# wei-zeng98/piano-a2s

Measured on AMD Instinct MI355X. Metric: training clips/sec (12 s, 5-bar), higher is better.
Workload: dtype f32

## Files before the change

### include/a2s.h

```cpp
#ifndef A2S_H
#define A2S_H
#include <stddef.h>
#include <stdint.h>
#ifdef __cplusplus
extern "C" {
#endif

#define A2S_OK 0
#define A2S_ERR_ARG (-1)
#define A2S_ERR_HIP (-2)
#define A2S_ERR_WORKSPACE (-3)

const char* a2s_last_error(void);
int a2s_version(void);
long long a2s_launch_count(void);

int a2s_gemm_f32(void* stream, int M, int N, int K, float alpha, const float* A, long sAm, long sAk,
                 const float* B, long sBk, long sBn, float beta, float* C, long ldc, const float* bias, int act,
                 int batch, long bsA, long bsB, long bsC, int splitk, float* workspace, size_t workspace_bytes);
int a2s_gemm_f32_affine(void* stream, int M, int N, int K, float alpha, const float* A, long sAm, long sAk, const float* B, long sBk,
                        long sBn, float beta, float* C, long ldc, const float* bias, int act, int batch, long bsA, long bsB, long bsC,
                        int splitk, float* workspace, size_t workspace_bytes, const float* a_scale, const float* a_shift, int a_period,
                        const float* b_scale, const float* b_shift, int b_period);
int a2s_gemm_f32_bnstats(void* stream, int M, int N, int K, const float* A, long sAm, long sAk, const float* B, long sBk, long sBn, float* C, long ldc,
                         const float* y, const float* mean, const float* invstd, const float* scale, const float* shift, int period, float* partial);
int a2s_gemm_f32_affine_scaled(void* stream, int M, int N, int K, float alpha, const float* A, long sAm, long sAk, const float* B, long sBk,
                               long sBn, float beta, float* C, long ldc, const float* bias, int act, int batch, long bsA, long bsB, long bsC,
                               int splitk, float* workspace, size_t workspace_bytes, const float* a_scale, const float* a_shift, int a_period,
                               const float* b_scale, const float* b_shift, int b_period, const float* a_absmax, const float* b_absmax);
int a2s_gemm_f32_bnstats_scaled(void* stream, int M, int N, int K, const float* A, long sAm, long sAk, const float* B, long sBk, long sBn, float* C, long ldc,
                                const float* y, const float* mean, const float* invstd, const float* scale, const float* shift, int period, float* partial,
                                const float* a_absmax, const float* b_absmax);
int a2s_linear_dgrad_bnstats(void* stream, int M, int N, int K, const float* dz, long lda, const float* Wt, float* da, long ldc, const float* y,
                             const float* mean, const float* invstd, const float* scale, const float* shift, int period, float* partial,
                             const float* dz_absmax, const float* w_absmax, float* workspace, size_t workspace_bytes, float* da_absmax_out);
int a2s_linear_fwd(void* stream, int M, int N, int K, const float* y, long lda, const float* W, float* z, long ldc, const float* scale, const float* shift,
                   int period, const float* y_absmax, const float* w_absmax, float* workspace, size_t workspace_bytes);
int a2s_linear_fwd_eligible(int M, int N, int K, int period);
int a2s_linear_wgrad(void* stream, int M, int N, int K, const float* dz, long ldz, const float* y, long lda, float* G, long ldg, const float* scale,
                     const float* shift, int period, const float* dz_absmax, const float* y_absmax, float* workspace, size_t workspace_bytes);
size_t a2s_linear_wgrad_ws_bytes(int M, int K);
int a2s_linear_wgrad_eligible(int M, int N, int K, int period);
int a2s_tallk_wgrad(void* stream, int M, int Np, int K, const float* P, long ldp, const float* A, long lda, float* G, long ldg, int transposed, float* bias,
                    const float* p_absmax, const float* a_absmax, float* workspace, size_t workspace_bytes);
size_t a2s_tallk_wgrad_ws_bytes(int M, int Np, int K);
int a2s_tallk_wgrad_eligible(int M, int Np, int K, long ldp, long lda, long ldg, int transposed);
size_t a2s_linear_dgrad_ws_bytes(int N, int K);
int a2s_linear_dgrad_blocks(int M);
int a2s_linear_dgrad_eligible(int M, int N, int K, int period);
int a2s_absmax(void* stream, const float* x, long n, float* out);
int a2s_gemm_bnstats_blocks(int M, int period);
size_t a2s_gemm_workspace_bytes(int M, int N, int batch, int splitk);
int a2s_gemm_pick_splitk(int M, int N, int K, int batch);
void a2s_gemm_debug_tile(int cfg);
int a2s_debug_set(const char* key, int value);
int a2s_debug_get(const char* key);
int a2s_env_check(void);
int a2s_persist_abort_latch(void* device_word);

int a2s_conv3x3(void* stream, const float* x, const float* w, float* y, const float* in_scale, const float* in_shift,
                float* stat_partial, int B, int T, int F, int Cin, int Cout, int flip, float* workspace);
int a2s_conv3x3_ranged(void* stream, const float* x, const float* w, float* y, const float* in_scale, const float* in_shift, const float* in_absmax,
                       float* stat_partial, float* out_absmax, int B, int T, int F, int Cin, int Cout, float* workspace);
int a2s_conv3x3_stat_blocks(int B, int T, int F, int Cin);
int a2s_conv3x3_dgrad_bnstats(void* stream, const float* dy, const float* w, float* g, const float* yl, const float* yl_mean, const float* yl_invstd,
                              const float* yl_scale, const float* yl_shift, float* stat_partial, int B, int T, int F, int Cin, int Cout,
                              float* workspace);
int a2s_bn_bwd_from_partial(void* stream, const float* g, const float* x, const float* mean, const float* invstd, const float* scale, const float* shift,
                            float* dgamma, float* dbeta, float* dx , const float* partial, int nblocks, float* c12, long rows, int C, int F);
int a2s_conv3x3_dgrad_bnstats_scaled(void* stream, const float* dy, const float* w, float* g, const float* yl, const float* yl_mean, const float* yl_invstd,
                                     const float* yl_scale, const float* yl_shift, float* stat_partial, int B, int T, int F, int Cin, int Cout,
                                     float* workspace, const float* dy_absmax);
int a2s_conv3x3_dgrad_bnstats_ranged(void* stream, const float* dy, const float* w, float* g, const float* yl, const float* yl_mean, const float* yl_invstd,
                                     const float* yl_scale, const float* yl_shift, float* stat_partial, int B, int T, int F, int Cin, int Cout,
                                     float* workspace, const float* dy_absmax, float* g_absmax_out);
int a2s_bn_bwd_from_partial_amax(void* stream, const float* g, const float* x, const float* mean, const float* invstd, const float* scale, const float* shift,
                                 float* dgamma, float* dbeta, float* dx, const float* partial, int nblocks, float* c12, long rows, int C, int F,
                                 float* dx_absmax);
size_t a2s_conv3x3_workspace_floats(int Cin);
// ... 300 lines not shown
```

### piano_a2s_amd/csrc/a2s_api.hip

```cpp
#define A2S_SWITCHES_IMPL
#include "a2s_internal.h"

thread_local char a2s_err_msg[512] = {0};
long long a2s_launch_counter = 0;

#define ST ((hipStream_t)stream)

extern "C" {

const char* a2s_last_error(void) { return a2s_err_msg; }
int a2s_version(void) { return 1; }
long long a2s_launch_count(void) { return __atomic_load_n(&a2s_launch_counter, __ATOMIC_RELAXED); }

int a2s_gemm_f32(void* stream, int M, int N, int K, float alpha, const float* A, long sAm, long sAk, const float* B, long sBk,
                 long sBn, float beta, float* C, long ldc, const float* bias, int act, int batch, long bsA, long bsB, long bsC,
                 int splitk, float* workspace, size_t workspace_bytes) {
    return a2s_gemm_impl(ST, M, N, K, alpha, A, sAm, sAk, B, sBk, sBn, beta, C, ldc, bias, act, batch, bsA, bsB, bsC, splitk,
                         workspace, workspace_bytes);
}
int a2s_gemm_f32_affine(void* stream, int M, int N, int K, float alpha, const float* A, long sAm, long sAk, const float* B, long sBk,
                        long sBn, float beta, float* C, long ldc, const float* bias, int act, int batch, long bsA, long bsB, long bsC,
                        int splitk, float* workspace, size_t workspace_bytes, const float* a_scale, const float* a_shift, int a_period,
                        const float* b_scale, const float* b_shift, int b_period) {
    return a2s_gemm_affine_impl(ST, M, N, K, alpha, A, sAm, sAk, B, sBk, sBn, beta, C, ldc, bias, act, batch, bsA, bsB, bsC, splitk,
// ... 7 lines not shown
    return a2s_gemm_affine_impl(ST, M, N, K, alpha, A, sAm, sAk, B, sBk, sBn, beta, C, ldc, bias, act, batch, bsA, bsB, bsC, splitk,
                                workspace, workspace_bytes, a_scale, a_shift, a_period, b_scale, b_shift, b_period,
                                nullptr, nullptr, nullptr, nullptr, nullptr, nullptr, 0, 1, a_absmax, b_absmax);
}
int a2s_gemm_f32_bnstats_scaled(void* stream, int M, int N, int K, const float* A, long sAm, long sAk, const float* B, long sBk, long sBn, float* C, long ldc,
                                const float* y, const float* mean, const float* invstd, const float* scale, const float* shift, int period, float* partial,
                                const float* a_absmax, const float* b_absmax) {
    return a2s_gemm_affine_impl(ST, M, N, K, 1.f, A, sAm, sAk, B, sBk, sBn, 0.f, C, ldc, nullptr, 0, 1, 0, 0, 0, 1, nullptr, 0,
                                nullptr, nullptr, 0, nullptr, nullptr, 0, y, mean, invstd, scale, shift, partial, period, 1, a_absmax, b_absmax);
}
int a2s_absmax(void* stream, const float* x, long n, float* out) { return a2s_absmax_impl(ST, x, n, out); }
int a2s_linear_dgrad_bnstats(void* stream, int M, int N, int K, const float* dz, long lda, const float* Wt, float* da, long ldc, const float* y,
                             const float* mean, const float* invstd, const float* scale, const float* shift, int period, float* partial,
                             const float* dz_absmax, const float* w_absmax, float* workspace, size_t workspace_bytes, float* da_absmax_out) {
    return a2s_linear_dgrad_bnstats_impl(ST, M, N, K, dz, lda, Wt, 1, K, da, ldc, y, mean, invstd, scale, shift, period, partial, dz_absmax, w_absmax,
                                         workspace, workspace_bytes, da_absmax_out);
}
size_t a2s_linear_dgrad_ws_bytes(int N, int K) { return a2s_linear_dgrad_ws_bytes_impl(N, K); }
int a2s_linear_fwd(void* stream, int M, int N, int K, const float* y, long lda, const float* W, float* z, long ldc, const float* scale, const float* shift,
                   int period, const float* y_absmax, const float* w_absmax, float* workspace, size_t workspace_bytes) {
    return a2s_linear_fwd_impl(ST, M, N, K, y, lda, W, z, ldc, scale, shift, period, y_absmax, w_absmax, workspace, workspace_bytes);
}
int a2s_linear_wgrad(void* stream, int M, int N, int K, const float* dz, long ldz, const float* y, long lda, float* G, long ldg, const float* scale,
                     const float* shift, int period, const float* dz_absmax, const float* y_absmax, float* workspace, size_t workspace_bytes) {
    return a2s_linear_wgrad_impl(ST, M, N, K, dz, ldz, y, lda, G, ldg, scale, shift, period, dz_absmax, y_absmax, workspace, workspace_bytes);
}
size_t a2s_linear_wgrad_ws_bytes(int M, int K) { return a2s_linear_wgrad_ws_bytes_impl(M, K); }
int a2s_linear_wgrad_eligible(int M, int N, int K, int period) { return a2s_linear_wgrad_ok(M, N, K, 256, 4, 4, period, nullptr, nullptr, nullptr) ? 1 : 0; }
int a2s_tallk_wgrad(void* stream, int M, int Np, int K, const float* P, long ldp, const float* A, long lda, float* G, long ldg, int transposed, float* bias,
                    const float* p_absmax, const float* a_absmax, float* workspace, size_t workspace_bytes) {
    return a2s_tallk_wgrad_impl(ST, M, Np, K, P, ldp, A, lda, G, ldg, transposed, bias, p_absmax, a_absmax, workspace, workspace_bytes);
}
size_t a2s_tallk_wgrad_ws_bytes(int M, int Np, int K) { return a2s_tallk_wgrad_ws_bytes_impl(M, Np, K); }
int a2s_tallk_wgrad_eligible(int M, int Np, int K, long ldp, long lda, long ldg, int transposed) {
    return a2s_tallk_wgrad_ok(M, Np, K, ldp, lda, ldg, transposed, nullptr, nullptr, nullptr, nullptr) ? 1 : 0;
}
int a2s_linear_fwd_eligible(int M, int N, int K, int period) { return a2s_linear_fwd_ok(M, N, K, 4, 4, period, nullptr, nullptr, nullptr) ? 1 : 0; }
int a2s_linear_dgrad_blocks(int M) { return a2s_linear_dgrad_blocks_impl(M); }
int a2s_linear_dgrad_eligible(int M, int N, int K, int period) {
    return a2s_linear_dgrad_ok(M, N, K, 4, 1, K, 4, period, nullptr, nullptr, nullptr, nullptr) ? 1 : 0;
}
int a2s_gemm_f32_bnstats(void* stream, int M, int N, int K, const float* A, long sAm, long sAk, const float* B, long sBk, long sBn, float* C, long ldc,
                         const float* y, const float* mean, const float* invstd, const float* scale, const float* shift, int period, float* partial) {
    return a2s_gemm_affine_impl(ST, M, N, K, 1.f, A, sAm, sAk, B, sBk, sBn, 0.f, C, ldc, nullptr, 0, 1, 0, 0, 0, 1, nullptr, 0,
                                nullptr, nullptr, 0, nullptr, nullptr, 0, y, mean, invstd, scale, shift, partial, period, 0, nullptr, nullptr);
}
int a2s_gemm_bnstats_blocks(int M, int period) { return a2s_cdiv(M, 128) * a2s_gemm_bnstats_slots(period); }
size_t a2s_gemm_workspace_bytes(int M, int N, int batch, int splitk) { return a2s_gemm_workspace_bytes_impl(M, N, batch, splitk); }
int a2s_gemm_pick_splitk(int M, int N, int K, int batch) { return a2s_gemm_pick_splitk_impl(M, N, K, batch); }
void a2s_gemm_debug_tile(int cfg) { a2s_gemm_debug_tile_impl(cfg); }
size_t a2s_note_step_workspace_floats(int H, int E) { return a2s_note_step_workspace_floats_impl(H, E); }
int a2s_debug_set(const char* key, int value) {
    if (!key) return A2S_ERR_ARG;
    const int id = a2s_switch_find(key);
    if (id >= 0) { a2s_switch_store(id, value); return A2S_OK; }
    if (!strcmp(key, "attn_deferred_fast")) { a2s_attn_deferred_fast = value ? 1 : 0; return A2S_OK; }
    if (!strcmp(key, "tallk_wgrad")) { a2s_tallk_wgrad_on = value ? 1 : 0; return A2S_OK; }
    if (!strcmp(key, "tallk_wgrad_max_splits")) { a2s_tallk_wgrad_max_splits = value > 0 ? value : 0; return A2S_OK; }
    if (!strcmp(key, "gemm_tile")) { a2s_gemm_debug_tile_impl(value); return A2S_OK; }
    snprintf(a2s_err_msg, sizeof(a2s_err_msg), "a2s_debug_set: unknown key %s", key);
    return A2S_ERR_ARG;
}
int a2s_env_check(void) {
    if (const char* e = a2s_switch_env_error()) A2S_FAIL(A2S_ERR_ARG, "%s: expected a decimal number >= 0", e);
    return A2S_OK;
}

int a2s_persist_abort_latch(void* device_word) { a2s_persist_latch_set(device_word); return A2S_OK; }

int a2s_debug_get(const char* key) {
    if (!key) return -1;
    const int id = a2s_switch_find(key);
    if (id == A2S_SW_attn_pair_fused_rows) return a2s_attn_pair_fused_rows();
    if (id >= 0) return a2s_sw((a2s_switch)id);
    if (!strcmp(key, "attn_pair_launches")) return (int)a2s_attn_pair_launches();
    if (!strcmp(key, "attn_pair_bwd_launches")) return (int)a2s_attn_pair_bwd_launches();
    if (!strcmp(key, "attn_deferred_fast")) return a2s_attn_deferred_fast;
    if (!strcmp(key, "tallk_wgrad")) return a2s_tallk_wgrad_on;
    if (!strcmp(key, "tallk_wgrad_max_splits")) return a2s_tallk_wgrad_max_splits;
    if (!strcmp(key, "tallk_wgrad_launches")) return (int)a2s_tallk_wgrad_launches();
    if (!strcmp(key, "attn_dk_ahead_launches")) return (int)a2s_attn_dk_ahead_launches();
    if (!strcmp(key, "attn_denc_launches")) return (int)a2s_attn_denc_launches();
    if (!strcmp(key, "dec_mid_launches")) return a2s_dec_mid_launches();
    if (!strcmp(key, "dec_cmb_launches")) return a2s_dec_cmb_launches();
    if (!strcmp(key, "dec_persist_launches")) return a2s_dec_persist_launches();
    if (!strcmp(key, "edit_distance_launches")) return (int)a2s_edit_distance_launches();
    if (!strcmp(key, "conv_rows16_c20_launches")) return (int)a2s_conv_rows16_c20_launches();
    if (!strcmp(key, "device_cus")) return a2s_device_geometry().cus;
    if (!strcmp(key, "device_xccs")) return a2s_device_geometry().xccs;
    return -1;
}

int a2s_conv3x3(void* stream, const float* x, const float* w, float* y, const float* in_scale, const float* in_shift,
                float* stat_partial, int B, int T, int F, int Cin, int Cout, int flip, float* workspace) {
    return a2s_conv3x3_impl(ST, x, w, y, in_scale, in_shift, stat_partial, B, T, F, Cin, Cout, flip, workspace, nullptr, nullptr, nullptr, nullptr, nullptr, nullptr,
                            nullptr, nullptr);
}
int a2s_conv3x3_ranged(void* stream, const float* x, const float* w, float* y, const float* in_scale, const float* in_shift, const float* in_absmax,
                       float* stat_partial, float* out_absmax, int B, int T, int F, int Cin, int Cout, float* workspace) {
    return a2s_conv3x3_impl(ST, x, w, y, in_scale, in_shift, stat_partial, B, T, F, Cin, Cout, 0, workspace, nullptr, nullptr, nullptr, nullptr, nullptr, nullptr,
                            in_absmax, out_absmax);
}
int a2s_conv3x3_dgrad_bnstats(void* stream, const float* dy, const float* w, float* g, const float* yl, const float* yl_mean, const float* yl_invstd,
                              const float* yl_scale, const float* yl_shift, float* stat_partial, int B, int T, int F, int Cin, int Cout,
                              float* workspace) {
    if (!yl) { snprintf(a2s_err_msg, sizeof(a2s_err_msg), "conv3x3_dgrad_bnstats: yl is required"); return A2S_ERR_ARG; }
    return a2s_conv3x3_impl(ST, dy, w, g, nullptr, nullptr, stat_partial, B, T, F, Cin, Cout, 1, workspace, yl, yl_mean, yl_invstd, yl_scale, yl_shift, nullptr, nullptr, nullptr);
}
int a2s_conv3x3_dgrad_bnstats_scaled(void* stream, const float* dy, const float* w, float* g, const float* yl, const float* yl_mean, const float* yl_invstd,
                                     const float* yl_scale, const float* yl_shift, float* stat_partial, int B, int T, int F, int Cin, int Cout,
                                     float* workspace, const float* dy_absmax) {
    if (!yl) { snprintf(a2s_err_msg, sizeof(a2s_err_msg), "conv3x3_dgrad_bnstats_scaled: yl is required"); return A2S_ERR_ARG; }
    return a2s_conv3x3_impl(ST, dy, w, g, nullptr, nullptr, stat_partial, B, T, F, Cin, Cout, 1, workspace, yl, yl_mean, yl_invstd, yl_scale, yl_shift, dy_absmax, nullptr, nullptr);
// ... 384 lines not shown
```

### piano_a2s_amd/csrc/a2s_internal.h

```cpp
#pragma once
#include "a2s_common.h"
#include "../../include/a2s.h"
#include "a2s_switches.h"

static inline int a2s_attn_pair_fused_rows(void) {
    const int cap = a2s_sw(A2S_SW_dec_fused_max_rows), v = a2s_sw(A2S_SW_attn_pair_fused_rows);
    return v < cap ? v : cap;
}
static inline unsigned a2s_persist_dbg(void) {
    return (a2s_sw(A2S_SW_persist_force_agent) ? PERSIST_DBG_FORCE_AGENT : 0u) | (a2s_sw(A2S_SW_persist_inject_abort) ? PERSIST_DBG_INJECT_ABORT : 0u);
}

int a2s_absmax_impl(hipStream_t st, const float* x, long n, float* out);
size_t a2s_gemm_workspace_bytes_impl(int M, int N, int batch, int splitk);
int a2s_gemm_pick_splitk_impl(int M, int N, int K, int batch);
int a2s_gemm_bnstats_slots(int period);
void a2s_gemm_debug_tile_impl(int cfg);
int a2s_gemm_affine_impl(hipStream_t st, int M, int N, int K, float alpha, const float* A, long sAm, long sAk,
    const float* B, long sBk, long sBn, float beta, float* C, long ldc, const float* bias, int act,
    int batch, long bsA, long bsB, long bsC, int splitk, float* ws, size_t ws_bytes,
    const float* a_scale, const float* a_shift, int a_period, const float* b_scale, const float* b_shift, int b_period,
    const float* ep_y, const float* ep_mean, const float* ep_invstd, const float* ep_scale, const float* ep_shift,
    float* ep_partial, int ep_period, int two_term, const float* a_absmax, const float* b_absmax);
int a2s_gemm_impl(hipStream_t st, int M, int N, int K, float alpha, const float* A, long sAm, long sAk,
    const float* B, long sBk, long sBn, float beta, float* C, long ldc, const float* bias, int act,
    int batch, long bsA, long bsB, long bsC, int splitk, float* ws, size_t ws_bytes);

size_t a2s_linear_dgrad_ws_bytes_impl(int N, int K);
int a2s_linear_dgrad_blocks_impl(int M);
bool a2s_linear_dgrad_ok(int M, int N, int K, long lda, long sBk, long sBn, long ldc, int period, const void* A, const void* B, const void* C, const void* y);
int a2s_linear_dgrad_bnstats_impl(hipStream_t st, int M, int N, int K, const float* A, long lda, const float* Wt, long sBk, long sBn, float* C, long ldc,
    const float* ep_y, const float* mean, const float* invstd, const float* scale, const float* shift, int period,
    float* partial, const float* a_absmax, const float* b_absmax, float* ws, size_t ws_bytes, float* c_absmax_out);
bool a2s_linear_fwd_ok(int M, int N, int K, long lda, long ldc, int period, const void* A, const void* W, const void* C);
int a2s_linear_fwd_impl(hipStream_t st, int M, int N, int K, const float* A, long lda, const float* W, float* C, long ldc, const float* a_scale,
    const float* a_shift, int period, const float* a_absmax, const float* w_absmax, float* ws, size_t ws_bytes);
size_t a2s_linear_wgrad_ws_bytes_impl(int M, int K);
bool a2s_linear_wgrad_ok(int M, int N, int K, long ldz, long lda, long ldg, int period, const void* dz, const void* A, const void* G);
int a2s_linear_wgrad_impl(hipStream_t st, int M, int N, int K, const float* dz, long ldz, const float* A, long lda, float* G, long ldg, const float* a_scale,
    const float* a_shift, int period, const float* dz_absmax, const float* a_absmax, float* ws, size_t ws_bytes);
extern int a2s_tallk_wgrad_on;
extern int a2s_tallk_wgrad_max_splits;
long a2s_tallk_wgrad_launches(void);
size_t a2s_tallk_wgrad_ws_bytes_impl(int M, int Np, int K);
bool a2s_tallk_wgrad_ok(int M, int Np, int K, long ldp, long lda, long ldg, int transposed, const void* P, const void* A, const void* G, const void* bias);
int a2s_tallk_wgrad_impl(hipStream_t st, int M, int Np, int K, const float* P, long ldp, const float* A, long lda, float* G, long ldg, int transposed,
    float* bias, const float* p_absmax, const float* a_absmax, float* ws, size_t ws_bytes);

int a2s_act_bound_impl(hipStream_t st, const float* scale, const float* shift, const float* absmax, int C, float* out);
size_t a2s_conv3x3_workspace_floats_impl(int Cin);
int a2s_conv3x3_impl(hipStream_t st, const float* x, const float* w, float* y, const float* in_scale,
    const float* in_shift, float* stat_partial, int B, int T, int F, int Cin, int Cout, int flip, float* ws,
    const float* yl, const float* yl_mean, const float* yl_invstd, const float* yl_scale, const float* yl_shift,
    const float* x_absmax, const float* in_absmax, float* out_absmax);
int a2s_conv3x3_stat_blocks_impl(int B, int T, int F, int Cin);
int a2s_bn_finalize_impl(hipStream_t st, const float* partial, int nblocks, int C, double count, const float* gamma,
    const float* beta, float* running_mean, float* running_var, long long* nbt, float* mean,
    float* invstd, float* scale, float* shift, float eps, float momentum, int training);
int a2s_bn_relu_apply_impl(hipStream_t st, const float* x, float* y, const float* scale, const float* shift, long n, int C, int F);
int a2s_col_stats_impl(hipStream_t st, const float* x, float* partial, long rows, int C, int rows_per_block);
int a2s_bn1d_relu_dropout_impl(hipStream_t st, const float* x, float* y, const float* scale, const float* shift,
    const uint8_t* mask, float inv_keep, long n, int C);
size_t a2s_conv3x3_wgrad_workspace_bytes_impl(int Cin, int Cout);
int a2s_conv3x3_wgrad_impl(hipStream_t st, const float* dy, const float* x, const float* in_scale, const float* in_shift, float* dW,
    float* ws, size_t ws_bytes, int B, int T, int F, int Cin, int Cout, const float* bn_y, const float* bn_mean,
    const float* bn_invstd, const float* bn_scale, const float* bn_shift, const float* bn_c12, float* dy_out,
    const float* dy_absmax, const float* act_absmax);
int a2s_bn_bwd_impl(hipStream_t st, const float* g, const float* x, const float* mean, const float* invstd, const float* scale,
    const float* shift, const uint8_t* mask, float inv_keep, float* dgamma, float* dbeta, float* dx, float* partial,
    float* c12, long rows, int C, int F, float* dx_absmax);
int a2s_bn_bwd_from_partial_impl(hipStream_t st, const float* g, const float* x, const float* mean, const float* invstd, const float* scale,
    const float* shift, float* dgamma, float* dbeta, float* dx, const float* partial, int nblocks, float* c12,
    long rows, int C, int F, float* dx_absmax);
int a2s_bn_bwd_stats_impl(hipStream_t st, const float* g, const float* x, const float* mean, const float* invstd, const float* scale,
    const float* shift, const uint8_t* mask, float inv_keep, float* partial, float* sums, long rows, int C, int F);
int a2s_bn_bwd_apply_impl(hipStream_t st, const float* g, const float* x, const float* mean, const float* invstd, const float* scale,
// ... 305 lines not shown
```

### piano_a2s_amd/csrc/a2s_linear.hip

```cpp
#include "a2s_internal.h"

#define LIN_BM 128
#define LIN_K 256
#define LIN_RS 288
#define LIN_NTH 512
#define LIN_LDS (2 * 2 * LIN_BM * LIN_RS)

typedef unsigned lu32x4 __attribute__((ext_vector_type(4)));

struct LinDgradArgs {
    const float* A; long lda;
    const unsigned char* planes;
    float* C; long ldc;
    const float* ep_y;
    const float* mean; const float* invstd; const float* scale; const float* shift;
    float* partial;
    const float* a_absmax; const float* b_absmax;
    int M, N, period, channels;
    float* c_absmax_out;
};

__global__ __launch_bounds__(256) void lin_pack_planes_k(const float* __restrict__ W, long ld, int N, int K, const float* __restrict__ absmax,
                                                         unsigned char* __restrict__ out) {
    const long id = (long)blockIdx.x * 256 + threadIdx.x;
// ... 580 lines not shown
    if (M < 1 || K < LIN_BM || K % LIN_BM) return 0;
    const size_t nsteps = 2 * (size_t)((M + 63) / 64);
    return nsteps * 16 * 2 * 1024 + (size_t)lin_wgrad_splits(M, K) * 256 * K * sizeof(float);
}
bool a2s_linear_wgrad_ok(int M, int N, int K, long ldz, long lda, long ldg, int period, const void* dz, const void* A, const void* G) {
    return N == 256 && M >= 64 && K >= LIN_BM && K % LIN_BM == 0 && (period == 0 || (period % 4 == 0 && K % period == 0)) && lda % 4 == 0 && ldg % 4 == 0 && ldz >= 256 &&
           (((uintptr_t)dz | (uintptr_t)A | (uintptr_t)G) % 16 == 0);
}
int a2s_linear_wgrad_impl(hipStream_t st, int M, int N, int K, const float* dz, long ldz, const float* A, long lda, float* G, long ldg, const float* a_scale,
                          const float* a_shift, int period, const float* dz_absmax, const float* a_absmax, float* ws, size_t ws_bytes) {
    A2S_REQUIRE(dz && A && G && dz_absmax && ws && ((a_scale == nullptr) == (a_shift == nullptr)), "linear_wgrad: null argument");
    A2S_REQUIRE(a2s_linear_wgrad_ok(M, N, K, ldz, lda, ldg, a_scale ? period : 0, dz, A, G), "linear_wgrad: needs N = 256, K %% 128 == 0, period %% 4 == 0, 16-byte aligned rows");
    A2S_REQUIRE(((uintptr_t)ws % 16 == 0) && ws_bytes >= a2s_linear_wgrad_ws_bytes_impl(M, K), "linear_wgrad: workspace too small (%zu bytes needed)",
                a2s_linear_wgrad_ws_bytes_impl(M, K));
    const int nblk = (M + 63) / 64, nsteps = 2 * nblk, splits = lin_wgrad_splits(M, K);
    unsigned char* planes = reinterpret_cast<unsigned char*>(ws);
    float* partial = reinterpret_cast<float*>(planes + (size_t)nsteps * 16 * 2 * 1024);
    hipLaunchKernelGGL(lin_pack_dz_planes, dim3((unsigned)(((long)nsteps * 1024 + 255) / 256)), dim3(256), 0, st, dz, ldz, M, nsteps, dz_absmax, planes);
    A2S_CHECK_LAUNCH("lin_pack_dz_planes");
    LinWgradArgs a{A, lda, planes, partial, a_scale, a_shift, a_absmax, dz_absmax, M, K, a_scale ? period : K, nblk, (nblk + splits - 1) / splits, 0, 256, nullptr};
    hipLaunchKernelGGL(lin_wgrad_roles<false>, dim3(K / LIN_BM, splits), dim3(LIN_NTH), 0, st, a);
    A2S_CHECK_LAUNCH("lin_wgrad");
    const long n = 256L * K;
    hipLaunchKernelGGL(lin_wgrad_reduce<false>, dim3((unsigned)((n / 4 + 255) / 256)), dim3(256), 0, st, partial, splits, n, G, ldg, K, nullptr, nullptr);
    A2S_CHECK_LAUNCH("lin_wgrad_reduce");
    return A2S_OK;
}

#define TALLK_SLAB_BYTES (64u << 20)
int a2s_tallk_wgrad_on = 1;
int a2s_tallk_wgrad_max_splits = 0;
static long long g_tallk_launches = 0;
long a2s_tallk_wgrad_launches(void) { return (long)__atomic_load_n(&g_tallk_launches, __ATOMIC_RELAXED); }

static int tallk_splits(int M, int Np, int K) {
    const int tiles = (K / LIN_BM) * (Np / 256), nblk = (M + 63) / 64;
    int cus = a2s_device_geometry().cus;
    if (cus < 1) cus = 256;
    int s = cus / tiles;
    const size_t slab = (size_t)Np * K * sizeof(float);
    if ((size_t)s * slab > TALLK_SLAB_BYTES) s = (int)(TALLK_SLAB_BYTES / slab);
    if (s > nblk) s = nblk;
    if (a2s_tallk_wgrad_max_splits > 0 && s > a2s_tallk_wgrad_max_splits) s = a2s_tallk_wgrad_max_splits;
    return s < 1 ? 1 : s;
}
bool a2s_tallk_wgrad_ok(int M, int Np, int K, long ldp, long lda, long ldg, int transposed, const void* P, const void* A, const void* G, const void* bias) {
    return a2s_tallk_wgrad_on && M >= 64 && Np >= 256 && Np % 256 == 0 && Np <= 2048 && K >= LIN_BM && K % LIN_BM == 0 && K <= 4096 && ldp >= Np && lda >= K &&
           lda % 4 == 0 && ldg % 4 == 0 && ldg >= (transposed ? Np : K) && (((uintptr_t)P | (uintptr_t)A | (uintptr_t)G | (uintptr_t)bias) % 16 == 0);
}
size_t a2s_tallk_wgrad_ws_bytes_impl(int M, int Np, int K) {
    if (M < 1 || Np < 256 || Np % 256 || K < LIN_BM || K % LIN_BM) return 0;
    const size_t nsteps = 2 * (size_t)((M + 63) / 64), splits = (size_t)tallk_splits(M, Np, K);
    return (size_t)(Np / 256) * nsteps * 16 * 2 * 1024 + splits * Np * K * sizeof(float) + splits * K * sizeof(float);
}
int a2s_tallk_wgrad_impl(hipStream_t st, int M, int Np, int K, const float* P, long ldp, const float* A, long lda, float* G, long ldg, int transposed,
                         float* bias, const float* p_absmax, const float* a_absmax, float* ws, size_t ws_bytes) {
    A2S_REQUIRE(P && A && G && p_absmax && a_absmax && ws, "tallk_wgrad: null argument");
    A2S_REQUIRE(a2s_tallk_wgrad_ok(M, Np, K, ldp, lda, ldg, transposed, P, A, G, bias),
                "tallk_wgrad: needs M >= 64, Np %% 256 == 0, K %% 128 == 0, 16-byte aligned bases and rows (or the switch \"tallk_wgrad\" is off)");
    A2S_REQUIRE(((uintptr_t)ws % 16 == 0) && ws_bytes >= a2s_tallk_wgrad_ws_bytes_impl(M, Np, K), "tallk_wgrad: workspace too small (%zu bytes needed)",
                a2s_tallk_wgrad_ws_bytes_impl(M, Np, K));
    const int nblk = (M + 63) / 64, nsteps = 2 * nblk, splits = tallk_splits(M, Np, K), npb = Np / 256;
    const size_t plane_stride = (size_t)nsteps * 16 * 2 * 1024;
    unsigned char* planes = reinterpret_cast<unsigned char*>(ws);
    float* partial = reinterpret_cast<float*>(planes + npb * plane_stride);
    float* bias_partial = partial + (size_t)splits * Np * K;
    hipLaunchKernelGGL(lin_pack_dz_planes, dim3((unsigned)(((long)nsteps * 1024 + 255) / 256), npb), dim3(256), 0, st, P, ldp, M, nsteps, p_absmax, planes);
    A2S_CHECK_LAUNCH("lin_pack_dz_planes");
    LinWgradArgs a{A, lda, planes, partial, nullptr, nullptr, a_absmax, p_absmax, M, K, K, nblk, (nblk + splits - 1) / splits, (long)plane_stride, Np,
                   bias ? bias_partial : nullptr};
    if (bias) hipLaunchKernelGGL(lin_wgrad_roles<true>, dim3(K / LIN_BM, splits, npb), dim3(LIN_NTH), 0, st, a);
    else hipLaunchKernelGGL(lin_wgrad_roles<false>, dim3(K / LIN_BM, splits, npb), dim3(LIN_NTH), 0, st, a);
    A2S_CHECK_LAUNCH("lin_wgrad (tall-K)");
    const long n = (long)Np * K, nthreads = (n + (bias ? K : 0)) / 4;
    const dim3 rgrid((unsigned)((nthreads + 255) / 256));
    if (transposed) hipLaunchKernelGGL(lin_wgrad_reduce<true>, rgrid, dim3(256), 0, st, partial, splits, n, G, ldg, K, bias ? bias_partial : nullptr, bias);
    else hipLaunchKernelGGL(lin_wgrad_reduce<false>, rgrid, dim3(256), 0, st, partial, splits, n, G, ldg, K, bias ? bias_partial : nullptr, bias);
    A2S_CHECK_LAUNCH("lin_wgrad_reduce");
    __atomic_fetch_add(&g_tallk_launches, 1LL, __ATOMIC_RELAXED);
    return A2S_OK;
}
```

### piano_a2s_amd/engine_bwd.py

```python
import ctypes as C
import os
import threading
from collections import namedtuple

import torch

from . import hip
from .conv_bwd_plan import CHANS, ConvBwdFlags, plan_convstack_bwd
from .dec_bwd_plan import dim, plan_note_decoder_bwd, plan_staff_issue
from .spec import SOS, VOCAB_SIZE


def _ptr(t, off=0):
    return C.c_void_p(t.data_ptr() + 4 * off)


_COLSUM_WS = {}


def _colsum(x, ld, out, rows, ncol, x_off=0, out_off=0, beta=1.0):
    ws = None
    if rows >= 2048:
        key = (x.device, torch.cuda.current_stream().cuda_stream, threading.get_ident())
        ws = _COLSUM_WS.get(key)
# ... 411 lines not shown
        return G




def backward(eng, S, grad_outputs, grad_ready=None, loss_total=None):
    from .engine import group_views, run_clip_groups
    sv = eng.saved
    assert sv["training"], "backward needs a forward run with training=True (batch statistics / saved activations)"
    dev = sv["enc_out"].device
    clip_groups = sv.get("clip_groups") or [(0, sv["shape"][0])]
    ctx = Backward(eng, S, sv["shape"], dev, clip_groups, sv.get("concurrent"), sv.get("bar_major"))
    dts, dkey, dup, dlo = [g.contiguous() for g in grad_outputs]

    def group(gidx):
        b0, b1 = clip_groups[gidx]
        if ctx.bar_major:
            dup_g, dlo_g = group_views(dup, clip_groups, gidx), group_views(dlo, clip_groups, gidx)
        else:
            dup_g, dlo_g = dup[b0:b1], dlo[b0:b1]
        ctx.decoder_group(gidx, sv["groups"][gidx], dts[b0:b1], dkey[b0:b1], dup_g, dlo_g)

    run_clip_groups(dev, [lambda gi=gi: group(gi) for gi in range(len(clip_groups))])
    if loss_total is not None:
        ctx.flat_full[ctx.total:].copy_(loss_total.reshape(1))
    return ctx.finish(grad_ready)


def _weight_grad_stream(dev):
    from .engine import group_stream
    return group_stream(dev, 1)


def _encoder_bwd(eng, S, G, es, dEnc, d_hidden, B, T):
    L = hip.lib()
    H = eng.cfg["hidden_size"]
    dev = dEnc.device
    W = S["encoder.fc.weight"]
    dpre = torch.empty_like(d_hidden)
    hip.check(L.a2s_ew_act_bwd(hip.stream(), hip._p(d_hidden), hip._p(es["hidden"]), hip._p(dpre), dpre.numel(), 2), "tanh bwd")
    dhn = []
    for l in (0, 1):
        for half, hfin in enumerate((es["finals"][2 * l], es["finals"][2 * l + 1])):
            d = torch.empty((B, H), device=dev)
            hip.gemm(dpre, 2 * H, 1, W, 2 * H, 1, d, H, B, H, H, a_off=l * H, b_off=half * H)
            hip.gemm(dpre, 1, 2 * H, hfin, H, 1, G["encoder.fc.weight"], 2 * H, H, H, B, beta=1.0, a_off=l * H, c_off=half * H)
            dhn.append(d)
        _colsum(dpre, 2 * H, G["encoder.fc.bias"], B, H, x_off=l * H)
    gws = [hip.gemm_workspace(B, dev), hip.gemm_workspace(B, dev)]
    in_amax = hip.absmax(es["layers"][0]["in"])
    dout = dEnc
    for layer in (1, 0):
        ls = es["layers"][layer]
        inp = ls["in"]
        I = inp.shape[1]
        out = ls["out"]
        dX = torch.empty((B * T, I), device=dev)
        from .engine import encoder_streams, fork_on_streams
        streams = encoder_streams(dev, B)

        def direction(d, sfx):
            dgi = torch.empty((B, T, 3 * H), device=dev)
            dghs = torch.empty((B, T, 3 * H), device=dev)
            dgh_first, dhbuf, dgh_tmp = torch.empty((B, 3 * H), device=dev), torch.empty((2, B, H), device=dev), torch.empty((B, 3 * H), device=dev)
            ranges, valid = torch.empty(2, device=dev), C.c_int(0)
            if L.a2s_debug_get(b"tallk_wgrad") > 0:
                hip.check(L.a2s_gru_seq_bwd_ranged(hip.stream(), _ptr(dout, d * H), T * 2 * H, 2 * H, _ptr(out, d * H), T * 2 * H, 2 * H, hip._p(ls["dirs"][d]["gates"]),
                                                   hip._p(S[f"encoder.gru.weight_hh_{sfx}"]), hip._p(dhn[2 * layer + d]), hip._p(dgi), hip._p(dghs), hip._p(dgh_first),
                                                   hip._p(dhbuf), hip._p(dgh_tmp), B, T, H, d, hip._p(gws[d]), gws[d].numel() * 4, hip._p(ranges), C.byref(valid)),
                          "a2s_gru_seq_bwd_ranged")
            else:
                hip.check(L.a2s_gru_seq_bwd(hip.stream(), _ptr(dout, d * H), T * 2 * H, 2 * H, _ptr(out, d * H), T * 2 * H, 2 * H, hip._p(ls["dirs"][d]["gates"]),
                                            hip._p(S[f"encoder.gru.weight_hh_{sfx}"]), hip._p(dhn[2 * layer + d]), hip._p(dgi), hip._p(dghs), hip._p(dgh_first),
                                            hip._p(dhbuf), hip._p(dgh_tmp), B, T, H, d, hip._p(gws[d]), gws[d].numel() * 4), "a2s_gru_seq_bwd")
            return (dgi, dghs, dgh_first, dhbuf, dgh_tmp, ranges if valid.value else None)

        res = fork_on_streams(dev, streams, [lambda d=d, sfx=sfx: direction(d, sfx) for d, sfx in enumerate((f"l{layer}", f"l{layer}_reverse"))])()
        dgi_amax = []
        for d, sfx in enumerate((f"l{layer}", f"l{layer}_reverse")):
            dgi2 = res[d][0].view(B * T, 3 * H)
            Wih = S[f"encoder.gru.weight_ih_{sfx}"]
            ranges = res[d][5]
            tt = (ranges[0:1] if ranges is not None else hip.absmax(dgi2), hip.absmax(Wih))
            dgi_amax.append(tt[0])
            if L.a2s_debug_get(b"gemm_bf16x3") > 0:
                hip.gemm(dgi2, 3 * H, 1, Wih.t().contiguous(), 1, 3 * H, dX, I, B * T, I, 3 * H, beta=0.0 if d == 0 else 1.0, two_term=tt)
            else:
                hip.gemm(dgi2, 3 * H, 1, Wih, I, 1, dX, I, B * T, I, 3 * H, beta=0.0 if d == 0 else 1.0, two_term=tt)
        wg = _weight_grad_stream(dev)
        ev = torch.cuda.Event()
        ev.record()
        wg.wait_event(ev)
        for d, sfx in enumerate((f"l{layer}", f"l{layer}_reverse")):
            dgi, dghs, dgh_first, ranges = res[d][0], res[d][1], res[d][2], res[d][5]
            for t in (dgi, dghs, dgh_first, dgi_amax[d], in_amax, ranges):
                if t is not None:
                    t.record_stream(wg)
            with torch.cuda.stream(wg):
                dgi2, dghs2 = dgi.view(B * T, 3 * H), dghs.view(B * T, 3 * H)
                x_bound = in_amax if layer == 0 else hip.one(dev)
                if not hip.tallk_wgrad(inp, 0, I, dgi2, 0, 3 * H, G[f"encoder.gru.weight_ih_{sfx}"], 0, I, B * T, I, 3 * H, x_bound, dgi_amax[d],
                                       transposed=True, bias=G[f"encoder.gru.bias_ih_{sfx}"]):
                    _linear_bwd(inp, S[f"encoder.gru.weight_ih_{sfx}"], dgi2, G, f"encoder.gru.weight_ih_{sfx}", f"encoder.gru.bias_ih_{sfx}",
                                dy_amax=dgi_amax[d], x_bound=x_bound)
                dghs_amax = ranges[1:2] if ranges is not None else hip.absmax(dghs2)
                if not hip.tallk_wgrad(out, d * H, 2 * H, dghs2, 0, 3 * H, G[f"encoder.gru.weight_hh_{sfx}"], 0, H, B * T, H, 3 * H,
                                       hip.one(dev), dghs_amax, transposed=True, bias=G[f"encoder.gru.bias_hh_{sfx}"]):
                    sk = L.a2s_gemm_pick_splitk(3 * H, H, B * T, 1)
                    hip.gemm(dghs2, 1, 3 * H, out, 2 * H, 1, G[f"encoder.gru.weight_hh_{sfx}"], H, 3 * H, H, B * T, beta=1.0, splitk=sk, b_off=d * H,
                             two_term=(dghs_amax, hip.one(dev)))
                    _colsum(dghs2, 3 * H, G[f"encoder.gru.bias_hh_{sfx}"], B * T, 3 * H)
                _colsum(dgh_first, 3 * H, G[f"encoder.gru.bias_hh_{sfx}"], B, 3 * H)
        dout = dX.view(B, T, I)
    return dout


_FUSE_BN_APPLY = False
_FUSE_BN_APPLY_L1 = True
_DGRAD_BNSTATS = True
_SYNC_FUSED = True
_LIN_WGRAD_AT = "before"
_FUSE_BN_ROWS = os.environ.get("A2S_FUSE_BN_ROWS", "1") != "0"
GradIn = namedtuple("GradIn", "g partial amax", defaults=(None, None))


def _bn_bwd(source, eng, G, name, gin, x, bn, dims, mask=None, dx=None, amax=None):
    dgamma, dbeta = G[name + ".weight"], G[name + ".bias"]
    if source in ("own", "partial"):
        return hip.bn_bwd(gin.g, x, bn, mask, dgamma, dbeta, dx, dims, amax, gin.partial if source == "partial" else None)
    import torch.distributed as dist
    return hip.bn_bwd_sync(gin.g, x, bn, mask, dgamma, dbeta, dims, eng.bn_counts[name], dist.all_reduce, gin.partial if source == "sync_partial" else None)


# ... 65 lines not shown
```

### piano_a2s_amd/hip.py

```python
import ctypes as C
import os
import threading

import numpy as np
import torch

from .abi import PROTOTYPES, STRUCTS, A2SError
from .build import LIB

LIB = os.environ.get("A2S_LIB", LIB)

NoteDecArgs, NoteDecBwdArgs, BeamArgs, AlignArgs = (STRUCTS[n] for n in ("a2s_note_dec_args", "a2s_note_dec_bwd_args", "a2s_beam_args", "a2s_align_args"))
_lib = None


def set_row_plan(a, active):
    active = active or {}
    for field, key in (("clip_order", "order"), ("clip_rank", "rank"), ("row_until", "until"), ("row_list", "row_list")):
        setattr(a, field, active[key].data_ptr() if active.get(key) is not None else None)
    for field, key in (("n_active", "n_active"), ("m_active", "m_active"), ("n_rows_active", "n_rows_active")):
        host = active.get(key) if (key != "n_rows_active" or active.get("row_list") is not None) else None
        setattr(a, field, C.cast(host, C.c_void_p).value if host is not None else None)
    a.n_clips = active.get("n_clips", 0)

# ... 1038 lines not shown
    if own:
        nb = L.a2s_linear_dgrad_ws_bytes(K, Cf)
        Wt, ws, amax = W.t().contiguous(), _f32(dz, nb // 4), torch.zeros(1, dtype=torch.float32, device=dz.device)
        check(L.a2s_linear_dgrad_bnstats(stream(), rows, K, Cf, _p(dz), Cf, _p(Wt), _p(da), K, _p(y), *map(_p, bn), F, _p(part), _p(dz_absmax), _p(w_absmax), _p(ws), nb,
                                         _p(amax)), "a2s_linear_dgrad_bnstats")
        return (part, nblk), amax
    wb, s_bk, s_bn = (W.t().contiguous(), 1, Cf) if L.a2s_debug_get(b"gemm_bf16x3") > 0 else (W, K, 1)
    check(L.a2s_gemm_f32_bnstats_scaled(stream(), rows, K, Cf, _p(dz), Cf, 1, _p(wb), s_bk, s_bn, _p(da), K, _p(y), *map(_p, bn), F, _p(part), _p(dz_absmax), _p(w_absmax)),
          "a2s_gemm_f32_bnstats_scaled")
    return (part, nblk), None


_TALLK_WS = {}


def tallk_wgrad(P, p_off, ldp, A, a_off, lda, G, g_off, ldg, M, Np, K, p_absmax, a_absmax, transposed=False, bias=None):
    L = lib()
    if not hasattr(L, "a2s_tallk_wgrad_eligible"):
        return False
    pp, pa, pg = P.data_ptr() + 4 * p_off, A.data_ptr() + 4 * a_off, G.data_ptr() + 4 * g_off
    if (p_absmax is None or a_absmax is None or (pp | pa | pg | (bias.data_ptr() if bias is not None else 0)) % 16
            or not L.a2s_tallk_wgrad_eligible(M, Np, K, ldp, lda, ldg, int(transposed))):
        return False
    nb = L.a2s_tallk_wgrad_ws_bytes(M, Np, K)
    key = (A.device, torch.cuda.current_stream().cuda_stream, threading.get_ident())
    ws = _TALLK_WS.get(key)
    if ws is None or ws.numel() * 4 < nb:
        ws = _TALLK_WS[key] = torch.empty((nb + 3) // 4, dtype=torch.float32, device=A.device)
    check(L.a2s_tallk_wgrad(stream(), M, Np, K, C.c_void_p(pp), ldp, C.c_void_p(pa), lda, C.c_void_p(pg), ldg, int(transposed), _p(bias), _p(p_absmax), _p(a_absmax),
                            _p(ws), ws.numel() * 4), "a2s_tallk_wgrad")
    return True


def linear_forward_for_test(x, w, aff):
    period = aff[2]
    xmax = x.view(x.shape[0], -1, period).abs().amax(dim=(0, 2)).contiguous()
    return linear_forward(x, w, aff, act_bound(aff[0], aff[1], xmax), absmax(w))
```

Before: 639.0.

## Pack encoder GRU activation planes once and share across directions' weight grads

Splits the tall-K weight-gradient path into a separate pack step and a packed-wgrad step, exposed through new API entry points. In the encoder backward, the quantized planes of each layer's input and output activations are built once per backward pass and reused by both GRU directions. Layer 1's input planes alias layer 0's output planes. This removes repeated lin_pack_dz_planes launches and their reads of the activation tensors, in exchange for keeping extra cached plane buffers alive and relying on the aliasing checks made in plan().

```diff
diff --git a/include/a2s.h b/include/a2s.h
--- a/include/a2s.h
+++ b/include/a2s.h
@@ -45,6 +45,11 @@
                     const float* p_absmax, const float* a_absmax, float* workspace, size_t workspace_bytes);
 size_t a2s_tallk_wgrad_ws_bytes(int M, int Np, int K);
 int a2s_tallk_wgrad_eligible(int M, int Np, int K, long ldp, long lda, long ldg, int transposed);
+size_t a2s_tallk_pack_bytes(int rows, int cols);
+int a2s_tallk_pack(void* stream, const float* x, long col_off, long ld, int rows, int cols, const float* bound, void* planes);
+size_t a2s_tallk_wgrad_packed_ws_bytes(int M, int n_blocks, int K);
+int a2s_tallk_wgrad_packed(void* stream, int M, int K, const float* A, long lda, const void* planes, int n_blocks, float* G, long ldg, int transposed, float* bias,
+                           const float* p_absmax, const float* a_absmax, float* workspace, size_t workspace_bytes);
 size_t a2s_linear_dgrad_ws_bytes(int N, int K);
 int a2s_linear_dgrad_blocks(int M);
 int a2s_linear_dgrad_eligible(int M, int N, int K, int period);
diff --git a/piano_a2s_amd/csrc/a2s_api.hip b/piano_a2s_amd/csrc/a2s_api.hip
--- a/piano_a2s_amd/csrc/a2s_api.hip
+++ b/piano_a2s_amd/csrc/a2s_api.hip
@@ -63,6 +63,15 @@
     return a2s_tallk_wgrad_impl(ST, M, Np, K, P, ldp, A, lda, G, ldg, transposed, bias, p_absmax, a_absmax, workspace, workspace_bytes);
 }
 size_t a2s_tallk_wgrad_ws_bytes(int M, int Np, int K) { return a2s_tallk_wgrad_ws_bytes_impl(M, Np, K); }
+size_t a2s_tallk_pack_bytes(int rows, int cols) { return a2s_tallk_pack_bytes_impl(rows, cols); }
+int a2s_tallk_pack(void* stream, const float* x, long col_off, long ld, int rows, int cols, const float* bound, void* planes) {
+    return a2s_tallk_pack_impl(ST, x, col_off, ld, rows, cols, bound, planes);
+}
+size_t a2s_tallk_wgrad_packed_ws_bytes(int M, int n_blocks, int K) { return a2s_tallk_wgrad_packed_ws_bytes_impl(M, n_blocks, K); }
+int a2s_tallk_wgrad_packed(void* stream, int M, int K, const float* A, long lda, const void* planes, int n_blocks, float* G, long ldg, int transposed, float* bias,
+                           const float* p_absmax, const float* a_absmax, float* workspace, size_t workspace_bytes) {
+    return a2s_tallk_wgrad_packed_impl(ST, M, n_blocks, K, planes, A, lda, G, ldg, transposed, bias, p_absmax, a_absmax, workspace, workspace_bytes, true);
+}
 int a2s_tallk_wgrad_eligible(int M, int Np, int K, long ldp, long lda, long ldg, int transposed) {
     return a2s_tallk_wgrad_ok(M, Np, K, ldp, lda, ldg, transposed, nullptr, nullptr, nullptr, nullptr) ? 1 : 0;
 }
@@ -88,6 +97,7 @@
     if (!strcmp(key, "attn_deferred_fast")) { a2s_attn_deferred_fast = value ? 1 : 0; return A2S_OK; }
     if (!strcmp(key, "tallk_wgrad")) { a2s_tallk_wgrad_on = value ? 1 : 0; return A2S_OK; }
     if (!strcmp(key, "tallk_wgrad_max_splits")) { a2s_tallk_wgrad_max_splits = value > 0 ? value : 0; return A2S_OK; }
+    if (!strcmp(key, "tallk_pack_once")) { a2s_tallk_pack_once = value ? 1 : 0; return A2S_OK; }
     if (!strcmp(key, "gemm_tile")) { a2s_gemm_debug_tile_impl(value); return A2S_OK; }
     snprintf(a2s_err_msg, sizeof(a2s_err_msg), "a2s_debug_set: unknown key %s", key);
     return A2S_ERR_ARG;
@@ -110,6 +120,9 @@
     if (!strcmp(key, "tallk_wgrad")) return a2s_tallk_wgrad_on;
     if (!strcmp(key, "tallk_wgrad_max_splits")) return a2s_tallk_wgrad_max_splits;
     if (!strcmp(key, "tallk_wgrad_launches")) return (int)a2s_tallk_wgrad_launches();
+    if (!strcmp(key, "tallk_pack_once")) return a2s_tallk_pack_once;
+    if (!strcmp(key, "tallk_pack_launches")) return (int)a2s_tallk_pack_launches();
+    if (!strcmp(key, "tallk_packed_launches")) return (int)a2s_tallk_packed_launches();
     if (!strcmp(key, "attn_dk_ahead_launches")) return (int)a2s_attn_dk_ahead_launches();
     if (!strcmp(key, "attn_denc_launches")) return (int)a2s_attn_denc_launches();
     if (!strcmp(key, "dec_mid_launches")) return a2s_dec_mid_launches();
diff --git a/piano_a2s_amd/csrc/a2s_internal.h b/piano_a2s_amd/csrc/a2s_internal.h
--- a/piano_a2s_amd/csrc/a2s_internal.h
+++ b/piano_a2s_amd/csrc/a2s_internal.h
@@ -41,7 +41,15 @@
     const float* a_shift, int period, const float* dz_absmax, const float* a_absmax, float* ws, size_t ws_bytes);
 extern int a2s_tallk_wgrad_on;
 extern int a2s_tallk_wgrad_max_splits;
+extern int a2s_tallk_pack_once;
 long a2s_tallk_wgrad_launches(void);
+long a2s_tallk_pack_launches(void);
+long a2s_tallk_packed_launches(void);
+size_t a2s_tallk_pack_bytes_impl(int rows, int cols);
+int a2s_tallk_pack_impl(hipStream_t st, const float* x, long col_off, long ld, int rows, int cols, const float* bound, void* planes);
+size_t a2s_tallk_wgrad_packed_ws_bytes_impl(int M, int n_blocks, int K);
+int a2s_tallk_wgrad_packed_impl(hipStream_t st, int M, int n_blocks, int K, const void* planes, const float* A, long lda, float* G, long ldg, int transposed,
+                                float* bias, const float* p_absmax, const float* a_absmax, float* ws, size_t ws_bytes, bool callers_planes);
 size_t a2s_tallk_wgrad_ws_bytes_impl(int M, int Np, int K);
 bool a2s_tallk_wgrad_ok(int M, int Np, int K, long ldp, long lda, long ldg, int transposed, const void* P, const void* A, const void* G, const void* bias);
 int a2s_tallk_wgrad_impl(hipStream_t st, int M, int Np, int K, const float* P, long ldp, const float* A, long lda, float* G, long ldg, int transposed,
diff --git a/piano_a2s_amd/csrc/a2s_linear.hip b/piano_a2s_amd/csrc/a2s_linear.hip
--- a/piano_a2s_amd/csrc/a2s_linear.hip
+++ b/piano_a2s_amd/csrc/a2s_linear.hip
@@ -636,6 +636,10 @@
 int a2s_tallk_wgrad_max_splits = 0;
 static long long g_tallk_launches = 0;
 long a2s_tallk_wgrad_launches(void) { return (long)__atomic_load_n(&g_tallk_launches, __ATOMIC_RELAXED); }
+int a2s_tallk_pack_once = 1;
+static long long g_tallk_pack_launches = 0, g_tallk_packed_launches = 0;
+long a2s_tallk_pack_launches(void) { return (long)__atomic_load_n(&g_tallk_pack_launches, __ATOMIC_RELAXED); }
+long a2s_tallk_packed_launches(void) { return (long)__atomic_load_n(&g_tallk_packed_launches, __ATOMIC_RELAXED); }
 
 static int tallk_splits(int M, int Np, int K) {
     const int tiles = (K / LIN_BM) * (Np / 256), nblk = (M + 63) / 64;
@@ -652,27 +656,45 @@
     return a2s_tallk_wgrad_on && M >= 64 && Np >= 256 && Np % 256 == 0 && Np <= 2048 && K >= LIN_BM && K % LIN_BM == 0 && K <= 4096 && ldp >= Np && lda >= K &&
            lda % 4 == 0 && ldg % 4 == 0 && ldg >= (transposed ? Np : K) && (((uintptr_t)P | (uintptr_t)A | (uintptr_t)G | (uintptr_t)bias) % 16 == 0);
 }
+size_t a2s_tallk_pack_bytes_impl(int rows, int cols) {
+    if (rows < 1 || cols < 256 || cols % 256) return 0;
+    return (size_t)(cols / 256) * (2 * (size_t)((rows + 63) / 64)) * 16 * 2 * 1024;
+}
+int a2s_tallk_pack_impl(hipStream_t st, const float* x, long col_off, long ld, int rows, int cols, const float* bound, void* planes) {
+    A2S_REQUIRE(x && bound && planes, "tallk_pack: null argument");
+    A2S_REQUIRE(rows >= 64 && cols >= 256 && cols % 256 == 0 && cols <= 2048 && col_off >= 0 && ld >= col_off + cols &&
+                ((uintptr_t)(x + col_off) | (uintptr_t)planes) % 16 == 0,
+                "tallk_pack: needs rows >= 64, cols %% 256 == 0, the columns inside the row, 16-byte aligned first column and planes");
+    const int nsteps = 2 * ((rows + 63) / 64);
+    hipLaunchKernelGGL(lin_pack_dz_planes, dim3((unsigned)(((long)nsteps * 1024 + 255) / 256), cols / 256), dim3(256), 0, st, x + col_off, ld, rows, nsteps, bound,
+                       reinterpret_cast<unsigned char*>(planes));
+    A2S_CHECK_LAUNCH("lin_pack_dz_planes");
+    __atomic_fetch_add(&g_tallk_pack_launches, 1LL, __ATOMIC_RELAXED);
+    return A2S_OK;
+}
+size_t a2s_tallk_wgrad_packed_ws_bytes_impl(int M, int n_blocks, int K) {
+    if (M < 1 || n_blocks < 1 || K < LIN_BM || K % LIN_BM) return 0;
+    const size_t splits = (size_t)tallk_splits(M, n_blocks * 256, K);
+    return splits * n_blocks * 256 * K * sizeof(float) + splits * K * sizeof(float);
+}
 size_t a2s_tallk_wgrad_ws_bytes_impl(int M, int Np, int K) {
     if (M < 1 || Np < 256 || Np % 256 || K < LIN_BM || K % LIN_BM) return 0;
-    const size_t nsteps = 2 * (size_t)((M + 63) / 64), splits = (size_t)tallk_splits(M, Np, K);
-    return (size_t)(Np / 256) * nsteps * 16 * 2 * 1024 + splits * Np * K * sizeof(float) + splits * K * sizeof(float);
-}
-int a2s_tallk_wgrad_impl(hipStream_t st, int M, int Np, int K, const float* P, long ldp, const float* A, long lda, float* G, long ldg, int transposed,
-                         float* bias, const float* p_absmax, const float* a_absmax, float* ws, size_t ws_bytes) {
-    A2S_REQUIRE(P && A && G && p_absmax && a_absmax && ws, "tallk_wgrad: null argument");
-    A2S_REQUIRE(a2s_tallk_wgrad_ok(M, Np, K, ldp, lda, ldg, transposed, P, A, G, bias),
+    return a2s_tallk_pack_bytes_impl(M, Np) + a2s_tallk_wgrad_packed_ws_bytes_impl(M, Np / 256, K);
+}
+int a2s_tallk_wgrad_packed_impl(hipStream_t st, int M, int n_blocks, int K, const void* planes, const float* A, long lda, float* G, long ldg, int transposed,
+                                float* bias, const float* p_absmax, const float* a_absmax, float* ws, size_t ws_bytes, bool callers_planes) {
+    const int Np = n_blocks * 256;
+    A2S_REQUIRE(planes && A && G && p_absmax && a_absmax && ws, "tallk_wgrad: null argument");
+    A2S_REQUIRE(n_blocks >= 1 && a2s_tallk_wgrad_ok(M, Np, K, Np, lda, ldg, transposed, planes, A, G, bias),
                 "tallk_wgrad: needs M >= 64, Np %% 256 == 0, K %% 128 == 0, 16-byte aligned bases and rows (or the switch \"tallk_wgrad\" is off)");
-    A2S_REQUIRE(((uintptr_t)ws % 16 == 0) && ws_bytes >= a2s_tallk_wgrad_ws_bytes_impl(M, Np, K), "tallk_wgrad: workspace too small (%zu bytes needed)",
-                a2s_tallk_wgrad_ws_bytes_impl(M, Np, K));
-    const int nblk = (M + 63) / 64, nsteps = 2 * nblk, splits = tallk_splits(M, Np, K), npb = Np / 256;
+    A2S_REQUIRE(((uintptr_t)ws % 16 == 0) && ws_bytes >= a2s_tallk_wgrad_packed_ws_bytes_impl(M, n_blocks, K), "tallk_wgrad: workspace too small (%zu bytes needed)",
+                a2s_tallk_wgrad_packed_ws_bytes_impl(M, n_blocks, K));
+    const int nblk = (M + 63) / 64, nsteps = 2 * nblk, splits = tallk_splits(M, Np, K), npb = n_blocks;
     const size_t plane_stride = (size_t)nsteps * 16 * 2 * 1024;
-    unsigned char* planes = reinterpret_cast<unsigned char*>(ws);
-    float* partial = reinterpret_cast<float*>(planes + npb * plane_stride);
+    float* partial = ws;
     float* bias_partial = partial + (size_t)splits * Np * K;
-    hipLaunchKernelGGL(lin_pack_dz_planes, dim3((unsigned)(((long)nsteps * 1024 + 255) / 256), npb), dim3(256), 0, st, P, ldp, M, nsteps, p_absmax, planes);
-    A2S_CHECK_LAUNCH("lin_pack_dz_planes");
-    LinWgradArgs a{A, lda, planes, partial, nullptr, nullptr, a_absmax, p_absmax, M, K, K, nblk, (nblk + splits - 1) / splits, (long)plane_stride, Np,
-                   bias ? bias_partial : nullptr};
+    LinWgradArgs a{A, lda, reinterpret_cast<const unsigned char*>(planes), partial, nullptr, nullptr, a_absmax, p_absmax, M, K, K, nblk, (nblk + splits - 1) / splits,
+                   (long)plane_stride, Np, bias ? bias_partial : nullptr};
     if (bias) hipLaunchKernelGGL(lin_wgrad_roles<true>, dim3(K / LIN_BM, splits, npb), dim3(LIN_NTH), 0, st, a);
     else hipLaunchKernelGGL(lin_wgrad_roles<false>, dim3(K / LIN_BM, splits, npb), dim3(LIN_NTH), 0, st, a);
     A2S_CHECK_LAUNCH("lin_wgrad (tall-K)");
@@ -682,5 +704,18 @@
     else hipLaunchKernelGGL(lin_wgrad_reduce<false>, rgrid, dim3(256), 0, st, partial, splits, n, G, ldg, K, bias ? bias_partial : nullptr, bias);
     A2S_CHECK_LAUNCH("lin_wgrad_reduce");
     __atomic_fetch_add(&g_tallk_launches, 1LL, __ATOMIC_RELAXED);
+    if (callers_planes) __atomic_fetch_add(&g_tallk_packed_launches, 1LL, __ATOMIC_RELAXED);
     return A2S_OK;
 }
+int a2s_tallk_wgrad_impl(hipStream_t st, int M, int Np, int K, const float* P, long ldp, const float* A, long lda, float* G, long ldg, int transposed,
+                         float* bias, const float* p_absmax, const float* a_absmax, float* ws, size_t ws_bytes) {
+    A2S_REQUIRE(P && A && G && p_absmax && a_absmax && ws, "tallk_wgrad: null argument");
+    A2S_REQUIRE(a2s_tallk_wgrad_ok(M, Np, K, ldp, lda, ldg, transposed, P, A, G, bias),
+                "tallk_wgrad: needs M >= 64, Np %% 256 == 0, K %% 128 == 0, 16-byte aligned bases and rows (or the switch \"tallk_wgrad\" is off)");
+    A2S_REQUIRE(((uintptr_t)ws % 16 == 0) && ws_bytes >= a2s_tallk_wgrad_ws_bytes_impl(M, Np, K), "tallk_wgrad: workspace too small (%zu bytes needed)",
+                a2s_tallk_wgrad_ws_bytes_impl(M, Np, K));
+    const size_t pb = a2s_tallk_pack_bytes_impl(M, Np);
+    if (int rc = a2s_tallk_pack_impl(st, P, 0, ldp, M, Np, p_absmax, ws)) return rc;
+    return a2s_tallk_wgrad_packed_impl(st, M, Np / 256, K, ws, A, lda, G, ldg, transposed, bias, p_absmax, a_absmax,
+                                       reinterpret_cast<float*>(reinterpret_cast<unsigned char*>(ws) + pb), ws_bytes - pb, false);
+}
diff --git a/piano_a2s_amd/engine_bwd.py b/piano_a2s_amd/engine_bwd.py
--- a/piano_a2s_amd/engine_bwd.py
+++ b/piano_a2s_amd/engine_bwd.py
@@ -467,6 +467,40 @@
     return group_stream(dev, 1)
 
 
+class _EncoderPlanes:
+
+    def __init__(self, es, M, H, in_amax):
+        self.l0, self.l1 = es["layers"]
+        self.M, self.H, self.in_amax, self.planes = M, H, in_amax, {}
+
+    @staticmethod
+    def plan(es, M, H, in_amax):
+        L = hip.lib()
+        l0, l1 = es["layers"]
+        shared = l1["in"].data_ptr() == l0["out"].data_ptr() and l1["in"].shape[1] == 2 * H and l1["in"].is_contiguous() and l0["out"].is_contiguous()
+        if (not hasattr(L, "a2s_tallk_pack") or L.a2s_debug_get(b"tallk_pack_once") <= 0 or not shared or in_amax is None or H % 256
+                or any(t.data_ptr() % 16 for t in (l0["in"], l0["out"], l1["out"]))
+                or not all(L.a2s_tallk_wgrad_eligible(M, n, 3 * H, n, 3 * H, n, 1) for n in (l0["in"].shape[1], 2 * H, H))):
+            return None
+        return _EncoderPlanes(es, M, H, in_amax)
+
+    def get(self, kind, layer):
+        if kind == "in" and layer == 1:
+            kind, layer = "out", 0
+        if (kind, layer) not in self.planes:
+            M, H, x = self.M, self.H, (self.l0, self.l1)[layer][kind]
+            dev = x.device
+            if kind == "in":
+                I = x.shape[1]
+                pl = hip.tallk_pack(x, 0, I, M, I, self.in_amax, hip.tallk_planes(M, I // 256, dev, slot=("encoder", kind, layer)))
+            else:
+                pl = hip.tallk_planes(M, 2 * H // 256, dev, slot=("encoder", kind, layer))
+                for d in (0, 1):
+                    hip.tallk_pack(x, d * H, 2 * H, M, H, hip.one(dev), pl, block=d * (H // 256))
+            self.planes[kind, layer] = pl
+        return self.planes[kind, layer]
+
+
 def _encoder_bwd(eng, S, G, es, dEnc, d_hidden, B, T):
     L = hip.lib()
     H = eng.cfg["hidden_size"]
@@ -484,6 +518,7 @@
         _colsum(dpre, 2 * H, G["encoder.fc.bias"], B, H, x_off=l * H)
     gws = [hip.gemm_workspace(B, dev), hip.gemm_workspace(B, dev)]
     in_amax = hip.absmax(es["layers"][0]["in"])
+    planes = _EncoderPlanes.plan(es, B * T, H, in_amax)
     dout = dEnc
     for layer in (1, 0):
         ls = es["layers"][layer]
@@ -534,6 +569,16 @@
             with torch.cuda.stream(wg):
                 dgi2, dghs2 = dgi.view(B * T, 3 * H), dghs.view(B * T, 3 * H)
                 x_bound = in_amax if layer == 0 else hip.one(dev)
+                if planes is not None:
+                    ok = hip.tallk_wgrad_packed(planes.get("in", layer), I // 256, x_bound, dgi2, 0, 3 * H, G[f"encoder.gru.weight_ih_{sfx}"], 0, I, B * T, 3 * H,
+                                                dgi_amax[d], transposed=True, bias=G[f"encoder.gru.bias_ih_{sfx}"])
+                    dghs_amax = ranges[1:2] if ranges is not None else hip.absmax(dghs2)
+                    ok = ok and hip.tallk_wgrad_packed(planes.get("out", layer), H // 256, hip.one(dev), dghs2, 0, 3 * H, G[f"encoder.gru.weight_hh_{sfx}"], 0, H,
+                                                       B * T, 3 * H, dghs_amax, transposed=True, bias=G[f"encoder.gru.bias_hh_{sfx}"], block=d * (H // 256))
+                    if not ok:
+                        raise hip.A2SError("encoder backward: a product from shared planes was refused after _EncoderPlanes.plan found its shape eligible")
+                    _colsum(dgh_first, 3 * H, G[f"encoder.gru.bias_hh_{sfx}"], B, 3 * H)
+                    continue
                 if not hip.tallk_wgrad(inp, 0, I, dgi2, 0, 3 * H, G[f"encoder.gru.weight_ih_{sfx}"], 0, I, B * T, I, 3 * H, x_bound, dgi_amax[d],
                                        transposed=True, bias=G[f"encoder.gru.bias_ih_{sfx}"]):
                     _linear_bwd(inp, S[f"encoder.gru.weight_ih_{sfx}"], dgi2, G, f"encoder.gru.weight_ih_{sfx}", f"encoder.gru.bias_ih_{sfx}",
diff --git a/piano_a2s_amd/hip.py b/piano_a2s_amd/hip.py
--- a/piano_a2s_amd/hip.py
+++ b/piano_a2s_amd/hip.py
@@ -1094,6 +1094,44 @@
     return True
 
 
+def tallk_planes(rows, blocks, device, slot=None):
+    nb = lib().a2s_tallk_pack_bytes(rows, 256 * blocks)
+    if slot is None:
+        return torch.empty(nb, dtype=torch.uint8, device=device)
+    key = (torch.device(device), torch.cuda.current_stream().cuda_stream, threading.get_ident(), slot)
+    buf = _TALLK_WS.get(key)
+    if buf is None or buf.numel() < nb:
+        buf = _TALLK_WS[key] = torch.empty(nb, dtype=torch.uint8, device=device)
+    return buf
+
+
+def tallk_pack(x, col_off, ld, rows, cols, bound, planes, block=0):
+    L = lib()
+    off = block * L.a2s_tallk_pack_bytes(rows, 256)
+    if off + L.a2s_tallk_pack_bytes(rows, cols) > planes.numel():
+        raise ValueError("tallk_pack: the planes buffer is too small for these blocks")
+    check(L.a2s_tallk_pack(stream(), _p(x), col_off, ld, rows, cols, _p(bound), C.c_void_p(planes.data_ptr() + off)), "a2s_tallk_pack")
+    return planes
+
+
+def tallk_wgrad_packed(planes, n_blocks, p_absmax, A, a_off, lda, G, g_off, ldg, M, K, a_absmax, transposed=False, bias=None, block=0):
+    L = lib()
+    pa, pg = A.data_ptr() + 4 * a_off, G.data_ptr() + 4 * g_off
+    Np = 256 * n_blocks
+    if (a_absmax is None or (pa | pg | (bias.data_ptr() if bias is not None else 0)) % 16
+            or not L.a2s_tallk_wgrad_eligible(M, Np, K, Np, lda, ldg, int(transposed))):
+        return False
+    nb = L.a2s_tallk_wgrad_packed_ws_bytes(M, n_blocks, K)
+    key = (A.device, torch.cuda.current_stream().cuda_stream, threading.get_ident())
+    ws = _TALLK_WS.get(key)
+    if ws is None or ws.numel() * 4 < nb:
+        ws = _TALLK_WS[key] = torch.empty((nb + 3) // 4, dtype=torch.float32, device=A.device)
+    pp = planes.data_ptr() + block * L.a2s_tallk_pack_bytes(M, 256)
+    check(L.a2s_tallk_wgrad_packed(stream(), M, K, C.c_void_p(pa), lda, C.c_void_p(pp), n_blocks, C.c_void_p(pg), ldg, int(transposed), _p(bias), _p(p_absmax),
+                                   _p(a_absmax), _p(ws), ws.numel() * 4), "a2s_tallk_wgrad_packed")
+    return True
+
+
 def linear_forward_for_test(x, w, aff):
     period = aff[2]
     xmax = x.view(x.shape[0], -1, period).abs().amax(dim=(0, 2)).contiguous()
```

After: 640.3 (median of 6 runs). No clear change (+0.2%).
